# haiciyang/LaDiffCodec

Hardware: AMD Instinct MI355X
Metric: audio-sec decoded / wall-sec, 16kHz 3kbps 50-step DDPM (higher is better)
Workload: dtype bf16; 1 GPU; LaDiffCodec 3 kbps, diff_dims=256, enc_ratios 8 4, 50-step DDPM, batch=32x2.4 s utterances per GPU; global_batch=32, latent_len=1200, denoise_steps=50, rccl_ranks=1, batches_in_flight=1, parallelism=dp1 (utterance-sharded, no data-path collective)

## Files before the change

### ladiffcodec_amd/csrc/seanet.hip

```cpp
#include <type_traits>
#include "ldc_kernels.h"
#include "ldc_math.h"

namespace ldc {

__device__ __forceinline__ float sbf2f(unsigned short h) { return __uint_as_float(((unsigned)h) << 16); }
__device__ __forceinline__ unsigned short sf2bf(float f) { return hw_bf16(f); }
template <typename T>
__device__ __forceinline__ float sld(const void* p, size_t i);
template <>
__device__ __forceinline__ float sld<float>(const void* p, size_t i) { return reinterpret_cast<const float*>(p)[i]; }
template <>
__device__ __forceinline__ float sld<__bf16>(const void* p, size_t i) {
  return sbf2f(reinterpret_cast<const unsigned short*>(p)[i]);
}
template <typename T>
__device__ __forceinline__ void sst(void* p, size_t i, float v);
template <>
__device__ __forceinline__ void sst<float>(void* p, size_t i, float v) { reinterpret_cast<float*>(p)[i] = v; }
template <>
__device__ __forceinline__ void sst<__bf16>(void* p, size_t i, float v) {
  reinterpret_cast<unsigned short*>(p)[i] = sf2bf(v);
}

template <typename T>
__global__ __launch_bounds__(256) void conv_cin1_kernel(const float* x, void* y, const float* w, const float* bias,
                                                        int L, int Cout, int k) {
  extern __shared__ float sw[];
  for (int i = threadIdx.x; i < Cout * k; i += 256) sw[i] = w[i];
  for (int i = threadIdx.x; i < Cout; i += 256) sw[Cout * k + i] = bias ? bias[i] : 0.f;
  __syncthreads();
  const int b = blockIdx.y;
  const int pad = k - 1;
  const size_t total = (size_t)L * Cout;
  for (size_t idx = (size_t)blockIdx.x * 256 + threadIdx.x; idx < total; idx += (size_t)gridDim.x * 256) {
    const int l = (int)(idx / Cout), co = (int)(idx % Cout);
    float acc = sw[Cout * k + co];
    for (int t = 0; t < k; ++t) {
      int u = l + t - pad;
      if (u < 0) u = -u;
      if (u >= L) u = 2 * (L - 1) - u;
      acc += sw[co * k + t] * x[(size_t)b * L + u];
    }
    sst<T>(y, ((size_t)b * L + l) * Cout + co, acc);
  }
}

template <typename T>
__global__ __launch_bounds__(256) void conv_cin1_rows_kernel(const float* x, void* y, const float* w, const float* bias,
                                                             int L, int Cout, int k, int rows_per_block) {
  const int b = blockIdx.y;
  const int tpr = Cout / 4;
  const int c4 = (threadIdx.x % tpr) * 4, r0 = threadIdx.x / tpr, rstep = 256 / tpr;
  float wk[4][8], bv[4];
#pragma unroll
  for (int c = 0; c < 4; ++c) {
    bv[c] = bias ? bias[c4 + c] : 0.f;
#pragma unroll
    for (int t = 0; t < 8; ++t) wk[c][t] = t < k ? w[(c4 + c) * k + t] : 0.f;
  }
  const int pad = k - 1;
  const int lbeg = blockIdx.x * rows_per_block, lend = min(L, lbeg + rows_per_block);
  const float* xb = x + (size_t)b * L;
  for (int l = lbeg + r0; l < lend; l += rstep) {
    float xv[8];
#pragma unroll
    for (int t = 0; t < 8; ++t) {
      int u = l + t - pad;
      if (u < 0) u = -u;
      xv[t] = t < k ? xb[u] : 0.f;
    }
    float acc[4];
#pragma unroll
    for (int c = 0; c < 4; ++c) {
      acc[c] = bv[c];
#pragma unroll
      for (int t = 0; t < 8; ++t) acc[c] = fmaf(wk[c][t], xv[t], acc[c]);
    }
    const size_t o = ((size_t)b * L + l) * Cout + c4;
    if (sizeof(T) == 4) {
      *reinterpret_cast<float4*>(reinterpret_cast<float*>(y) + o) = make_float4(acc[0], acc[1], acc[2], acc[3]);
    } else {
      *reinterpret_cast<uint2*>(reinterpret_cast<unsigned short*>(y) + o) = make_uint2(hw_bf16x2(acc[0], acc[1]), hw_bf16x2(acc[2], acc[3]));
    }
  }
}

hipError_t launch_conv_cin1(int dt, const float* x, void* y, const float* w, const float* bias, int B, int L, int Cout,
                            int k, hipStream_t s, int* route_out) {
  if (L <= k - 1) return hipErrorInvalidValue;
  if (Cout % 4 == 0 && Cout <= 1024 && 256 % (Cout / 4) == 0 && k <= 8) {
    if (route_out) *route_out = CONV_ROUTE_CIN1_ROWS;
    const int rpb = 8 * (1024 / Cout);
    dim3 grid((L + rpb - 1) / rpb, B);
    if (dt == DT_F32) hipLaunchKernelGGL(conv_cin1_rows_kernel<float>, grid, dim3(256), 0, s, x, y, w, bias, L, Cout, k, rpb);
    else hipLaunchKernelGGL(conv_cin1_rows_kernel<__bf16>, grid, dim3(256), 0, s, x, y, w, bias, L, Cout, k, rpb);
    return hipGetLastError();
  }
  if (route_out) *route_out = CONV_ROUTE_CIN1_GENERIC;
  const size_t lds = (size_t)(Cout * k + Cout) * sizeof(float);
  int bx = (int)std::min<size_t>(((size_t)L * Cout + 255) / 256, 512);
  if (dt == DT_F32)
    hipLaunchKernelGGL(conv_cin1_kernel<float>, dim3(bx, B), dim3(256), lds, s, x, y, w, bias, L, Cout, k);
  else
    hipLaunchKernelGGL(conv_cin1_kernel<__bf16>, dim3(bx, B), dim3(256), lds, s, x, y, w, bias, L, Cout, k);
  return hipGetLastError();
}

__device__ __forceinline__ float sigmoid_acc(float v) { return 1.0f / (1.0f + expf(-v)); }

template <typename T, int H>
__global__ __launch_bounds__(4 * H) void lstm_reg_kernel(const void* pre, const float* w_hh, void* out, const void* skip,
                                                         const LstmSeq q) {
  constexpr int KS = H / 4;
  constexpr int KP = KS + 4;
  __shared__ __attribute__((aligned(16))) float sh[4 * KP];
  __shared__ float sg[4 * H];
  const int b = blockIdx.x, tid = threadIdx.x;
  const int rg = tid >> 2, g = tid & 3;
  float w[4][KS];
#pragma unroll
  for (int q = 0; q < 4; ++q)
#pragma unroll
    for (int k = 0; k < KS; k += 4) {
      const float4 v = *reinterpret_cast<const float4*>(w_hh + (size_t)(rg * 4 + q) * H + g * KS + k);
      w[q][k] = v.x; w[q][k + 1] = v.y; w[q][k + 2] = v.z; w[q][k + 3] = v.w;
    }
  const int row = tid;
  const bool resume = q.state && q.t0 > 0;
  float c = (resume && row < H) ? q.state[(size_t)b * 2 * H + H + row] : 0.f;
  float h_last = (resume && row < H) ? q.state[(size_t)b * 2 * H + row] : 0.f;
  if (row < H) sh[row + 4 * (row / KS)] = h_last;
  float p_next[4] = {0.f, 0.f, 0.f, 0.f};
  const size_t pre0 = (size_t)b * q.pre_bs, out0 = (size_t)b * q.out_bs, skip0 = (size_t)b * q.skip_bs;
  if (row < H) {
#pragma unroll
    for (int gq = 0; gq < 4; ++gq) p_next[gq] = sld<T>(pre, (pre0 + (size_t)q.t0 * q.pre_ts) * (4 * H) + gq * H + row);
  }
  float sk_next = (skip && row < H) ? sld<T>(skip, (skip0 + (size_t)q.t0 * q.skip_ts) * H + row) : 0.f;
  __syncthreads();
  for (int t = q.t0; t < q.t1; ++t) {
    const float p_cur[4] = {p_next[0], p_next[1], p_next[2], p_next[3]};
    const float sk = sk_next;
    if (t + 1 < q.t1 && row < H) {
#pragma unroll
      for (int gq = 0; gq < 4; ++gq) p_next[gq] = sld<T>(pre, (pre0 + (size_t)(t + 1) * q.pre_ts) * (4 * H) + gq * H + row);
      if (skip) sk_next = sld<T>(skip, (skip0 + (size_t)(t + 1) * q.skip_ts) * H + row);
    }
    typedef float f32x2 __attribute__((ext_vector_type(2)));
    f32x2 a01[4], a23[4];
#pragma unroll
    for (int q = 0; q < 4; ++q) { a01[q] = f32x2{0.f, 0.f}; a23[q] = f32x2{0.f, 0.f}; }
#pragma unroll
    for (int k = 0; k < KS; k += 4) {
      const float4 hv = *reinterpret_cast<const float4*>(&sh[g * KP + k]);
      const f32x2 h01 = {hv.x, hv.y}, h23 = {hv.z, hv.w};
#pragma unroll
      for (int q = 0; q < 4; ++q) {
        const f32x2 w01 = {w[q][k], w[q][k + 1]}, w23 = {w[q][k + 2], w[q][k + 3]};
        a01[q] = __builtin_elementwise_fma(w01, h01, a01[q]);
        a23[q] = __builtin_elementwise_fma(w23, h23, a23[q]);
      }
    }
#pragma unroll
    for (int q = 0; q < 4; ++q) {
      float v = (a01[q][0] + a01[q][1]) + (a23[q][0] + a23[q][1]);
      v += __int_as_float(__builtin_amdgcn_update_dpp(0, __float_as_int(v), 0xB1, 0xf, 0xf, true));
      v += __int_as_float(__builtin_amdgcn_update_dpp(0, __float_as_int(v), 0x4E, 0xf, 0xf, true));
      if (g == q) sg[rg * 4 + q] = v;
    }
    __syncthreads();
    if (row < H) {
      const float ig = fast_sigmoid(sg[row] + p_cur[0]), fg = fast_sigmoid(sg[H + row] + p_cur[1]);
      const float gg = fast_tanh(sg[2 * H + row] + p_cur[2]), og = fast_sigmoid(sg[3 * H + row] + p_cur[3]);
      c = fg * c + ig * gg;
      const float h = og * fast_tanh(c);
      h_last = h;
      sh[row + 4 * (row / KS)] = h;
      const size_t o = (out0 + (size_t)t * q.out_ts) * H + row;
      sst<T>(out, o, h + sk);
    }
    __syncthreads();
  }
  if (q.state && row < H) {
    q.state[(size_t)b * 2 * H + row] = h_last;
    q.state[(size_t)b * 2 * H + H + row] = c;
  }
}

template <typename T>
__global__ __launch_bounds__(1024) void lstm_stream_kernel(const void* pre, const float* w_km, void* out, const void* skip,
                                                           int T_len, int H) {
  extern __shared__ __attribute__((aligned(16))) float sm[];
  float* sh = sm;
  float* sg = sm + H;
  const int b = blockIdx.x, tid = threadIdx.x;
  const int G = 4 * H;
  for (int i = tid; i < H; i += 1024) sh[i] = 0.f;
  float c_state[4] = {0.f, 0.f, 0.f, 0.f};
  __syncthreads();
  for (int t = 0; t < T_len; ++t) {
    for (int row = tid; row < G; row += 1024) {
      float acc0 = 0.f, acc1 = 0.f;
      const float4* wp = reinterpret_cast<const float4*>(w_km) + row;
      for (int k4 = 0; k4 < H / 4; k4 += 2) {
        const float4 w0 = wp[(size_t)k4 * G];
        const float4 w1 = wp[(size_t)(k4 + 1) * G];
        const float4 h0 = *reinterpret_cast<const float4*>(&sh[4 * k4]);
        const float4 h1 = *reinterpret_cast<const float4*>(&sh[4 * k4 + 4]);
        acc0 += w0.x * h0.x + w0.y * h0.y + w0.z * h0.z + w0.w * h0.w;
        acc1 += w1.x * h1.x + w1.y * h1.y + w1.z * h1.z + w1.w * h1.w;
      }
      sg[row] = acc0 + acc1 + sld<T>(pre, ((size_t)b * T_len + t) * G + row);
    }
    __syncthreads();
    int ci = 0;
    for (int j = tid; j < H; j += 1024, ++ci) {
      const float ig = sigmoid_acc(sg[j]), fg = sigmoid_acc(sg[H + j]);
      const float gg = tanhf(sg[2 * H + j]), og = sigmoid_acc(sg[3 * H + j]);
      const float c = fg * c_state[ci] + ig * gg;
      c_state[ci] = c;
      const float h = og * tanhf(c);
      sh[j] = h;
      const size_t o = ((size_t)b * T_len + t) * H + j;
      sst<T>(out, o, skip ? h + sld<T>(skip, o) : h);
    }
    __syncthreads();
  }
}

constexpr int LSTM_COOP_SHARDS = 8;
constexpr int LSTM_COOP_SHARD_STRIDE = 16;
size_t lstm_coop_ws_bytes(int H) { return (size_t)2 * 32 * H * sizeof(float) + 256 * sizeof(unsigned); }

using f32x4 = __attribute__((ext_vector_type(4))) float;

template <typename T, int H>
__global__ __launch_bounds__(256) void lstm_coop_kernel(const void* pre, const float* w_hh, void* out, const void* skip,
                                                        int B, int T_len, float* hbuf, unsigned* sync, unsigned* host_flag) {
  constexpr int KW = H / 4;
  constexpr int NI = KW / 16;
  __shared__ float part[4][2][16][16];
  __shared__ int s_dead;
  const int tid = threadIdx.x, lane = tid & 63, w = tid >> 6;
  const int j = blockIdx.x, nb = gridDim.x;
  const int n = lane & 15, q = lane >> 4;
  const int MT = (B + 15) / 16;
  f32x4 breg[NI];
  {
    const size_t row = (size_t)(n >> 2) * H + 4 * j + (n & 3);
#pragma unroll
    for (int jj = 0; jj < NI; ++jj) breg[jj] = *reinterpret_cast<const f32x4*>(w_hh + row * H + w * KW + 16 * jj + 4 * q);
  }
  if (tid == 0) s_dead = 0;
  const int ob = tid >> 2, ou = tid & 3;
  const bool owner = tid < 4 * B;
  float c_state = 0.f;
  float pnext[4] = {0.f, 0.f, 0.f, 0.f};
  float sknext = 0.f;
  if (owner) {
#pragma unroll
    for (int g = 0; g < 4; ++g) pnext[g] = sld<T>(pre, ((size_t)ob * T_len) * (4 * H) + g * H + 4 * j + ou);
    if (skip) sknext = sld<T>(skip, ((size_t)ob * T_len) * H + 4 * j + ou);
  }
  __syncthreads();
  bool dead = false;
  int t = 0;
  for (; t < T_len; ++t) {
    f32x4 acc[2] = {{0.f, 0.f, 0.f, 0.f}, {0.f, 0.f, 0.f, 0.f}};
    if (t > 0) {
      if (w == 0) {
        const unsigned target = (unsigned)(t * (nb / LSTM_COOP_SHARDS));
        unsigned spins = 0;
        for (;;) {
          unsigned v = target;
          if (lane < LSTM_COOP_SHARDS) v = __hip_atomic_load(sync + lane * LSTM_COOP_SHARD_STRIDE, __ATOMIC_RELAXED, __HIP_MEMORY_SCOPE_AGENT);
          const unsigned flag = lane == 0 ? __hip_atomic_load(sync + 200, __ATOMIC_RELAXED, __HIP_MEMORY_SCOPE_AGENT) : 0u;
          if (__any(flag != 0u) || ++spins > 400000u) {
            if (lane == 0) { __hip_atomic_store(sync + 200, 1u, __ATOMIC_RELAXED, __HIP_MEMORY_SCOPE_AGENT); s_dead = 1; }
            break;
          }
          if (__all(v >= target)) break;
          __builtin_amdgcn_s_sleep(2);
        }
      }
      __syncthreads();
      if (s_dead) { dead = true; break; }
      const float* hp = hbuf + (size_t)((t + 1) & 1) * 32 * H;
      f32x4 areg[2][NI];
#pragma unroll
      for (int mt = 0; mt < 2; ++mt) {
        if (mt < MT) {
          const int item = min(mt * 16 + n, B - 1);
#pragma unroll
          for (int jj = 0; jj < NI; ++jj) {
            const float* src = hp + (size_t)item * H + w * KW + 16 * jj + 4 * q;
            asm volatile("global_load_dwordx4 %0, %1, off sc0 sc1" : "=v"(areg[mt][jj]) : "v"(src) : "memory");
          }
        }
      }
      asm volatile("s_waitcnt vmcnt(0)" ::: "memory");
#pragma unroll
      for (int mt = 0; mt < 2; ++mt)
        if (mt < MT) {
#pragma unroll
          for (int jj = 0; jj < NI; ++jj) asm volatile("" : "+v"(areg[mt][jj]));
        }
#pragma unroll
      for (int jj = 0; jj < NI; ++jj) {
#pragma unroll
        for (int e = 0; e < 4; ++e) {
          acc[0] = __builtin_amdgcn_mfma_f32_16x16x4f32(areg[0][jj][e], breg[jj][e], acc[0], 0, 0, 0);
          if (MT > 1) acc[1] = __builtin_amdgcn_mfma_f32_16x16x4f32(areg[1][jj][e], breg[jj][e], acc[1], 0, 0, 0);
        }
      }
    }
#pragma unroll
    for (int mt = 0; mt < 2; ++mt)
#pragma unroll
      for (int r = 0; r < 4; ++r) part[w][mt][4 * q + r][n] = acc[mt][r];
    __syncthreads();
    if (owner) {
      float gates[4];
#pragma unroll
      for (int g = 0; g < 4; ++g) {
        const int col = g * 4 + ou;
        gates[g] = pnext[g] + ((part[0][ob >> 4][ob & 15][col] + part[1][ob >> 4][ob & 15][col]) +
                               (part[2][ob >> 4][ob & 15][col] + part[3][ob >> 4][ob & 15][col]));
      }
      const float ig = sigmoid_acc(gates[0]), fg = sigmoid_acc(gates[1]);
      const float gg = tanhf(gates[2]), og = sigmoid_acc(gates[3]);
      c_state = fg * c_state + ig * gg;
      const float h = og * tanhf(c_state);
      __hip_atomic_store(hbuf + (size_t)(t & 1) * 32 * H + (size_t)ob * H + 4 * j + ou, h, __ATOMIC_RELAXED, __HIP_MEMORY_SCOPE_AGENT);
      asm volatile("s_waitcnt vmcnt(0)" ::: "memory");
      const size_t o = ((size_t)ob * T_len + t) * H + 4 * j + ou;
      sst<T>(out, o, h + sknext);
      if (t + 1 < T_len) {
#pragma unroll
        for (int g = 0; g < 4; ++g) pnext[g] = sld<T>(pre, ((size_t)ob * T_len + t + 1) * (4 * H) + g * H + 4 * j + ou);
        if (skip) sknext = sld<T>(skip, o + H);
      }
    }
    __syncthreads();
    if (tid == 0 && t + 1 < T_len)
      __hip_atomic_fetch_add(sync + (j % LSTM_COOP_SHARDS) * LSTM_COOP_SHARD_STRIDE, 1u, __ATOMIC_RELAXED, __HIP_MEMORY_SCOPE_AGENT);
  }
  if (dead && owner) {
    for (int tt = t; tt < T_len; ++tt) sst<T>(out, ((size_t)ob * T_len + tt) * H + 4 * j + ou, __builtin_nanf(""));
  }
  if (dead && tid == 0 && host_flag) __hip_atomic_store(host_flag, 1u, __ATOMIC_RELAXED, __HIP_MEMORY_SCOPE_SYSTEM);
}

template <int G>
__device__ __forceinline__ float dpp_sum_group(float v) {
  auto dpp = [](float x, auto ctrl) {
    return __int_as_float(__builtin_amdgcn_update_dpp(0, __float_as_int(x), decltype(ctrl)::value, 0xf, 0xf, true));
  };
  v += dpp(v, std::integral_constant<int, 0xB1>());
  v += dpp(v, std::integral_constant<int, 0x4E>());
  v += dpp(v, std::integral_constant<int, 0x141>());
  if (G >= 16) v += dpp(v, std::integral_constant<int, 0x140>());
  if (G >= 32) v += __shfl_xor(v, 16);
  if (G >= 64) v += __shfl_xor(v, 32);
  return v;
}

template <typename T, int H>
__global__ __launch_bounds__(1024) void lstm_xcd_kernel(const void* pre, const float* w_hh, void* out, const void* skip,
                                                        int B, int T_len, float* hbuf, unsigned* sync, unsigned* host_flag, unsigned long long* dbg = nullptr) {
  constexpr int NB = 16;
  constexpr int U = H / NB;
  constexpr int ROWS = 4 * U;
  constexpr int RPT = 2;
  constexpr int KSEG = 1024 / (ROWS / RPT);
  constexpr int KS = H / KSEG;
  constexpr int NV = KS / 4;
  constexpr int KPAD = KS >= 8 ? 4 : 0;
  __shared__ float sgate[2][ROWS];
  __shared__ __attribute__((aligned(16))) float sh[2][H + KPAD * KSEG];
  __shared__ int s_dead, s_rank;
  const int tid = threadIdx.x, lane = tid & 63, w = tid >> 6;
  const unsigned xcc = __builtin_amdgcn_s_getreg((20 << 0) | (0 << 6) | ((4 - 1) << 11)) & 7u;
  if (xcc != 0u) return;
  if (tid == 0) {
    s_rank = (int)__hip_atomic_fetch_add(sync + 202, 1u, __ATOMIC_RELAXED, __HIP_MEMORY_SCOPE_AGENT);
    s_dead = 0;
  }
  __syncthreads();
  const int j = s_rank;
  if (j >= NB) return;
  unsigned* flags = sync;
  const int rg = tid / KSEG, g = tid % KSEG;
  f32x4 wreg[RPT][NV];
#pragma unroll
  for (int q = 0; q < RPT; ++q) {
    const int r = rg * RPT + q;
    const size_t row = (size_t)(r / U) * H + (size_t)j * U + (r % U);
#pragma unroll
    for (int v = 0; v < NV; ++v) wreg[q][v] = *reinterpret_cast<const f32x4*>(w_hh + row * H + g * KS + 4 * v);
  }
  const int ob = tid / U, ou = tid % U;
  const bool owner = tid < U * B;
  float c_state = 0.f;
  float pnext[4] = {0.f, 0.f, 0.f, 0.f};
  float sknext = 0.f;
  if (owner) {
#pragma unroll
    for (int gg = 0; gg < 4; ++gg) pnext[gg] = sld<T>(pre, ((size_t)ob * T_len) * (4 * H) + gg * H + j * U + ou);
    if (skip) sknext = sld<T>(skip, ((size_t)ob * T_len) * H + j * U + ou);
  }
  bool dead = false;
  int t = 0;
  for (; t < T_len; ++t) {
    float dot[2][RPT];
#pragma unroll
    for (int q = 0; q < RPT; ++q) dot[0][q] = dot[1][q] = 0.f;
    unsigned long long st0 = 0, st1 = 0, st2 = 0, st3 = 0, st4 = 0, st5 = 0;
    const bool rec = dbg && j == 3 && tid == 0 && t >= 16 && t < 48;
    if (rec) st0 = __builtin_amdgcn_s_memtime();
    if (t > 0) {
      if (w == 0) {
        const unsigned long long t0 = wall_clock64();
        for (unsigned spins = 0;; ++spins) {
          const bool ok = lane >= NB || __hip_atomic_load(flags + lane, __ATOMIC_RELAXED, __HIP_MEMORY_SCOPE_AGENT) >= (unsigned)t;
          if (__all(ok)) break;
          if ((spins & 255u) == 255u) {
            const unsigned flag = lane == 0 ? __hip_atomic_load(sync + 200, __ATOMIC_RELAXED, __HIP_MEMORY_SCOPE_AGENT) : 0u;
            if (__any(flag != 0u) || wall_clock64() - t0 > 20000000ull) {
              if (lane == 0) { __hip_atomic_store(sync + 200, 1u, __ATOMIC_RELAXED, __HIP_MEMORY_SCOPE_AGENT); s_dead = 1; }
              break;
            }
          }
        }
      }
      __syncthreads();
      if (rec) st1 = __builtin_amdgcn_s_memtime();
      if (s_dead) { dead = true; break; }
      const float* hp = hbuf + (size_t)((t + 1) & 1) * 32 * H;
      if (tid < B * (H / 4)) {
        const int b = tid / (H / 4), v = tid % (H / 4);
        f32x4 hv;
        asm volatile("global_load_dwordx4 %0, %1, off sc1\n\ts_waitcnt vmcnt(0)" : "=&v"(hv) : "v"(hp + (size_t)b * H + 4 * v) : "memory");
        *reinterpret_cast<f32x4*>(&sh[b][4 * v + KPAD * ((4 * v) / KS)]) = hv;
      }
      __syncthreads();
      if (rec) st2 = __builtin_amdgcn_s_memtime();
#pragma unroll
      for (int b = 0; b < 2; ++b)
        if (b < B) {
#pragma unroll
          for (int v = 0; v < NV; ++v) {
            const f32x4 hv = *reinterpret_cast<const f32x4*>(&sh[b][g * (KS + KPAD) + 4 * v]);
#pragma unroll
            for (int q = 0; q < RPT; ++q)
#pragma unroll
              for (int e = 0; e < 4; ++e) dot[b][q] = fmaf(hv[e], wreg[q][v][e], dot[b][q]);
          }
        }
#pragma unroll
      for (int b = 0; b < 2; ++b)
        if (b < B) {
#pragma unroll
          for (int q = 0; q < RPT; ++q) dot[b][q] = dpp_sum_group<KSEG>(dot[b][q]);
        }
    }
    if (g == 0) {
#pragma unroll
      for (int q = 0; q < RPT; ++q) {
        sgate[0][rg * RPT + q] = dot[0][q];
        sgate[1][rg * RPT + q] = dot[1][q];
      }
    }
    __syncthreads();
    if (rec) st3 = __builtin_amdgcn_s_memtime();
    if (owner) {
      float gates[4];
#pragma unroll
      for (int gg = 0; gg < 4; ++gg) gates[gg] = pnext[gg] + sgate[ob][gg * U + ou];
      const float ig = sigmoid_acc(gates[0]), fg = sigmoid_acc(gates[1]);
      const float gv = tanhf(gates[2]), og = sigmoid_acc(gates[3]);
      c_state = fg * c_state + ig * gv;
      const float h = og * tanhf(c_state);
      asm volatile("global_store_dword %0, %1, off" ::"v"(hbuf + (size_t)(t & 1) * 32 * H + (size_t)ob * H + j * U + ou), "v"(h) : "memory");
      asm volatile("s_waitcnt vmcnt(0)" ::: "memory");
      if (rec) st4 = __builtin_amdgcn_s_memtime();
      const size_t o = ((size_t)ob * T_len + t) * H + j * U + ou;
      sst<T>(out, o, h + sknext);
      if (t + 1 < T_len) {
#pragma unroll
        for (int gg = 0; gg < 4; ++gg) pnext[gg] = sld<T>(pre, ((size_t)ob * T_len + t + 1) * (4 * H) + gg * H + j * U + ou);
        if (skip) sknext = sld<T>(skip, o + H);
      }
    }
    __syncthreads();
    if (tid == 0 && t + 1 < T_len) {
      asm volatile("global_store_dword %0, %1, off" ::"v"(flags + j), "v"((unsigned)(t + 1)) : "memory");
    }
    if (rec) { st5 = __builtin_amdgcn_s_memtime(); unsigned long long* o = dbg + (size_t)(t - 16) * 6; o[0] = st0; o[1] = st1; o[2] = st2; o[3] = st3; o[4] = st4; o[5] = st5; }
  }
  if (dead && owner) {
    for (int tt = t; tt < T_len; ++tt) sst<T>(out, ((size_t)ob * T_len + tt) * H + j * U + ou, __builtin_nanf(""));
  }
  if (dead && tid == 0 && host_flag) __hip_atomic_store(host_flag, 1u, __ATOMIC_RELAXED, __HIP_MEMORY_SCOPE_SYSTEM);
}

template <typename T>
static hipError_t lstm_coop_launch(const void* pre, const float* w_rm, void* out, const void* skip, int B, int T_len, int H,
                                   void* ws, unsigned* host_flag, int coop_launch, hipStream_t s) {
  float* hbuf = reinterpret_cast<float*>(ws);
  unsigned* sync = reinterpret_cast<unsigned*>(hbuf + (size_t)2 * 32 * H);
  const size_t esz = sizeof(T);
  for (int b0 = 0; b0 < B; b0 += 32) {
    const int nb = std::min(32, B - b0);
    hipError_t e = hipMemsetAsync(sync, 0, 256 * sizeof(unsigned), s);
    if (e != hipSuccess) return e;
    const char* p = reinterpret_cast<const char*>(pre) + (size_t)b0 * T_len * 4 * H * esz;
    char* o = reinterpret_cast<char*>(out) + (size_t)b0 * T_len * H * esz;
    const char* k = skip ? reinterpret_cast<const char*>(skip) + (size_t)b0 * T_len * H * esz : nullptr;
    const void* pp = p; void* oo = o; const void* kk = k; int nbv = nb, tl = T_len;
    void* args[] = {&pp, &w_rm, &oo, &kk, &nbv, &tl, &hbuf, &sync, &host_flag};
    const void* fn = H == 512 ? reinterpret_cast<const void*>(lstm_coop_kernel<T, 512>) : reinterpret_cast<const void*>(lstm_coop_kernel<T, 256>);
    if (coop_launch == 2 && nb <= 2) {
      const void* fx = H == 512 ? reinterpret_cast<const void*>(lstm_xcd_kernel<T, 512>) : reinterpret_cast<const void*>(lstm_xcd_kernel<T, 256>);
      static unsigned long long* dbg = nullptr;
      static int dbg_n = 0;
      if (getenv("LDC_LSTM_STAMPS") && !dbg) (void)hipMalloc((void**)&dbg, 32 * 6 * 8);
      void* args2[] = {&pp, &w_rm, &oo, &kk, &nbv, &tl, &hbuf, &sync, &host_flag, &dbg};
      e = hipLaunchKernel(fx, dim3(8 * 16), dim3(1024), args2, 0, s);
      if (dbg && ++dbg_n == 20) {
        (void)hipStreamSynchronize(s);
        unsigned long long hb[32 * 6];
        (void)hipMemcpy(hb, dbg, sizeof(hb), hipMemcpyDeviceToHost);
        double acc[6] = {0};
        for (int i = 1; i < 32; ++i) {
          acc[0] += (double)(hb[i * 6 + 1] - hb[i * 6 + 0]); acc[1] += (double)(hb[i * 6 + 2] - hb[i * 6 + 1]); acc[2] += (double)(hb[i * 6 + 3] - hb[i * 6 + 2]);
          acc[3] += (double)(hb[i * 6 + 4] - hb[i * 6 + 3]); acc[4] += (double)(hb[i * 6 + 5] - hb[i * 6 + 4]); acc[5] += (double)(hb[i * 6 + 0] - hb[(i - 1) * 6 + 0]);
        }
        fprintf(stderr, "[lstm_xcd] cycles per step: poll %.0f | h load %.0f | dot+reduce %.0f | gates+h store %.0f | rest+flag %.0f | step %.0f\n", acc[0] / 31, acc[1] / 31,
                acc[2] / 31, acc[3] / 31, acc[4] / 31, acc[5] / 31);
      }
    } else if (coop_launch == 1) e = hipLaunchCooperativeKernel(fn, dim3(H / 4), dim3(256), args, 0, s);
    else e = hipLaunchKernel(fn, dim3(H / 4), dim3(256), args, 0, s);
    if (e != hipSuccess) return e;
  }
  return hipSuccess;
}

bool lstm_coop_eligible(int H) { return H == 256 || H == 512; }
int lstm_xcd_resident(int H) {
  if (!lstm_coop_eligible(H)) return 0;
  const void* fn = H == 512 ? reinterpret_cast<const void*>(lstm_xcd_kernel<float, 512>) : reinterpret_cast<const void*>(lstm_xcd_kernel<float, 256>);
  int per_cu = 0, cus = 0, dev = 0;
  if (hipGetDevice(&dev) != hipSuccess || hipDeviceGetAttribute(&cus, hipDeviceAttributeMultiprocessorCount, dev) != hipSuccess ||
      hipOccupancyMaxActiveBlocksPerMultiprocessor(&per_cu, fn, 1024, 0) != hipSuccess) {
    (void)hipGetLastError();
    return 0;
  }
  if (cus % 8 != 0 || per_cu < 1) return 0;
  return per_cu * (cus / 8) / 16;
}

bool lstm_coop_resident(int H) {
  if (!lstm_coop_eligible(H)) return false;
  const void* fn = H == 512 ? reinterpret_cast<const void*>(lstm_coop_kernel<float, 512>) : reinterpret_cast<const void*>(lstm_coop_kernel<float, 256>);
  int dev = 0, per_cu = 0, cus = 0;
  if (hipGetDevice(&dev) != hipSuccess || hipDeviceGetAttribute(&cus, hipDeviceAttributeMultiprocessorCount, dev) != hipSuccess ||
      hipOccupancyMaxActiveBlocksPerMultiprocessor(&per_cu, fn, 256, 0) != hipSuccess) {
    (void)hipGetLastError();
    return false;
  }
  return (long long)std::max(0, per_cu - 1) * cus >= H / 4 || (long long)per_cu * cus >= 2 * (H / 4);
}

hipError_t launch_lstm_coop(int dt, const void* pre, const float* w_rm, void* out, const void* skip, int B, int T, int H,
                            void* ws, unsigned* host_flag, int coop_launch, hipStream_t s) {
  if (!lstm_coop_eligible(H)) return hipErrorInvalidValue;
  return dt == DT_F32 ? lstm_coop_launch<float>(pre, w_rm, out, skip, B, T, H, ws, host_flag, coop_launch, s)
                      : lstm_coop_launch<__bf16>(pre, w_rm, out, skip, B, T, H, ws, host_flag, coop_launch, s);
}

bool lstm_seq_supported(int H) { return H == 64 || H == 128; }

hipError_t launch_lstm_seq(int dt, const void* pre, const float* w_hh, void* out, const void* skip, int B, int H, const LstmSeq& q,
                           hipStream_t s) {
  if (!lstm_seq_supported(H) || q.t1 <= q.t0) return hipErrorInvalidValue;
  if (H == 64) {
    if (dt == DT_F32) hipLaunchKernelGGL((lstm_reg_kernel<float, 64>), dim3(B), dim3(256), 0, s, pre, w_hh, out, skip, q);
    else hipLaunchKernelGGL((lstm_reg_kernel<__bf16, 64>), dim3(B), dim3(256), 0, s, pre, w_hh, out, skip, q);
  } else {
    if (dt == DT_F32) hipLaunchKernelGGL((lstm_reg_kernel<float, 128>), dim3(B), dim3(512), 0, s, pre, w_hh, out, skip, q);
    else hipLaunchKernelGGL((lstm_reg_kernel<__bf16, 128>), dim3(B), dim3(512), 0, s, pre, w_hh, out, skip, q);
  }
  return hipGetLastError();
}

hipError_t launch_lstm_layer(int dt, const void* pre, const float* w_hh, void* out, const void* skip, int B, int T,
                             int H, hipStream_t s) {
  if (H % 8 || H > 4096) return hipErrorInvalidValue;
  if (H == 64 || H == 128) {
    LstmSeq q;
    q.t0 = 0; q.t1 = T; q.pre_bs = q.out_bs = q.skip_bs = T; q.pre_ts = q.out_ts = q.skip_ts = 1; q.state = nullptr;
    return launch_lstm_seq(dt, pre, w_hh, out, skip, B, H, q, s);
  } else {
    const size_t lds = (size_t)5 * H * sizeof(float);
    if (dt == DT_F32) hipLaunchKernelGGL(lstm_stream_kernel<float>, dim3(B), dim3(1024), lds, s, pre, w_hh, out, skip, T, H);
    else hipLaunchKernelGGL(lstm_stream_kernel<__bf16>, dim3(B), dim3(1024), lds, s, pre, w_hh, out, skip, T, H);
  }
  return hipGetLastError();
}

}
```

Measured before the change: 591.2 audio-s/wall-s.

## Remap LSTM gates per quad and double-buffer hidden state to drop a barrier

Reassigns the register-resident LSTM recurrent weights so each group of four lanes holds all four gates (i, f, g, o) of one hidden unit. The gate values are then exchanged with DPP quad broadcasts instead of going through a shared-memory gate buffer. The hidden state is double-buffered in LDS, which removes one of the two __syncthreads per timestep and the shared gate array. In exchange, all four lanes of a quad now compute the cell update redundantly, and the activation math is rewritten with a branch-free sigmoid/tanh that uses expf and a reciprocal.

```diff
diff --git a/ladiffcodec_amd/csrc/seanet.hip b/ladiffcodec_amd/csrc/seanet.hip
--- a/ladiffcodec_amd/csrc/seanet.hip
+++ b/ladiffcodec_amd/csrc/seanet.hip
@@ -114,38 +114,32 @@
                                                          const LstmSeq q) {
   constexpr int KS = H / 4;
   constexpr int KP = KS + 4;
-  __shared__ __attribute__((aligned(16))) float sh[4 * KP];
-  __shared__ float sg[4 * H];
+  __shared__ __attribute__((aligned(16))) float sh[2][4 * KP];
   const int b = blockIdx.x, tid = threadIdx.x;
-  const int rg = tid >> 2, g = tid & 3;
+  const int u = tid >> 2, g = tid & 3;
   float w[4][KS];
 #pragma unroll
   for (int q = 0; q < 4; ++q)
 #pragma unroll
     for (int k = 0; k < KS; k += 4) {
-      const float4 v = *reinterpret_cast<const float4*>(w_hh + (size_t)(rg * 4 + q) * H + g * KS + k);
+      const float4 v = *reinterpret_cast<const float4*>(w_hh + (size_t)(q * H + u) * H + g * KS + k);
       w[q][k] = v.x; w[q][k + 1] = v.y; w[q][k + 2] = v.z; w[q][k + 3] = v.w;
     }
-  const int row = tid;
   const bool resume = q.state && q.t0 > 0;
-  float c = (resume && row < H) ? q.state[(size_t)b * 2 * H + H + row] : 0.f;
-  float h_last = (resume && row < H) ? q.state[(size_t)b * 2 * H + row] : 0.f;
-  if (row < H) sh[row + 4 * (row / KS)] = h_last;
-  float p_next[4] = {0.f, 0.f, 0.f, 0.f};
+  float c = resume ? q.state[(size_t)b * 2 * H + H + u] : 0.f;
+  float h_last = resume ? q.state[(size_t)b * 2 * H + u] : 0.f;
+  if (g == 0) sh[0][u + 4 * (u / KS)] = h_last;
   const size_t pre0 = (size_t)b * q.pre_bs, out0 = (size_t)b * q.out_bs, skip0 = (size_t)b * q.skip_bs;
-  if (row < H) {
-#pragma unroll
-    for (int gq = 0; gq < 4; ++gq) p_next[gq] = sld<T>(pre, (pre0 + (size_t)q.t0 * q.pre_ts) * (4 * H) + gq * H + row);
-  }
-  float sk_next = (skip && row < H) ? sld<T>(skip, (skip0 + (size_t)q.t0 * q.skip_ts) * H + row) : 0.f;
+  float p_next = sld<T>(pre, (pre0 + (size_t)q.t0 * q.pre_ts) * (4 * H) + g * H + u);
+  float sk_next = (skip && g == 0) ? sld<T>(skip, (skip0 + (size_t)q.t0 * q.skip_ts) * H + u) : 0.f;
   __syncthreads();
-  for (int t = q.t0; t < q.t1; ++t) {
-    const float p_cur[4] = {p_next[0], p_next[1], p_next[2], p_next[3]};
+  int cur = 0;
+  for (int t = q.t0; t < q.t1; ++t, cur ^= 1) {
+    const float p_cur = p_next;
     const float sk = sk_next;
-    if (t + 1 < q.t1 && row < H) {
-#pragma unroll
-      for (int gq = 0; gq < 4; ++gq) p_next[gq] = sld<T>(pre, (pre0 + (size_t)(t + 1) * q.pre_ts) * (4 * H) + gq * H + row);
-      if (skip) sk_next = sld<T>(skip, (skip0 + (size_t)(t + 1) * q.skip_ts) * H + row);
+    if (t + 1 < q.t1) {
+      p_next = sld<T>(pre, (pre0 + (size_t)(t + 1) * q.pre_ts) * (4 * H) + g * H + u);
+      if (skip && g == 0) sk_next = sld<T>(skip, (skip0 + (size_t)(t + 1) * q.skip_ts) * H + u);
     }
     typedef float f32x2 __attribute__((ext_vector_type(2)));
     f32x2 a01[4], a23[4];
@@ -153,7 +147,7 @@
     for (int q = 0; q < 4; ++q) { a01[q] = f32x2{0.f, 0.f}; a23[q] = f32x2{0.f, 0.f}; }
 #pragma unroll
     for (int k = 0; k < KS; k += 4) {
-      const float4 hv = *reinterpret_cast<const float4*>(&sh[g * KP + k]);
+      const float4 hv = *reinterpret_cast<const float4*>(&sh[cur][g * KP + k]);
       const f32x2 h01 = {hv.x, hv.y}, h23 = {hv.z, hv.w};
 #pragma unroll
       for (int q = 0; q < 4; ++q) {
@@ -162,29 +156,33 @@
         a23[q] = __builtin_elementwise_fma(w23, h23, a23[q]);
       }
     }
+    float v[4];
 #pragma unroll
     for (int q = 0; q < 4; ++q) {
-      float v = (a01[q][0] + a01[q][1]) + (a23[q][0] + a23[q][1]);
-      v += __int_as_float(__builtin_amdgcn_update_dpp(0, __float_as_int(v), 0xB1, 0xf, 0xf, true));
-      v += __int_as_float(__builtin_amdgcn_update_dpp(0, __float_as_int(v), 0x4E, 0xf, 0xf, true));
-      if (g == q) sg[rg * 4 + q] = v;
+      v[q] = (a01[q][0] + a01[q][1]) + (a23[q][0] + a23[q][1]);
+      v[q] += __int_as_float(__builtin_amdgcn_update_dpp(0, __float_as_int(v[q]), 0xB1, 0xf, 0xf, true));
+      v[q] += __int_as_float(__builtin_amdgcn_update_dpp(0, __float_as_int(v[q]), 0x4E, 0xf, 0xf, true));
+    }
+    const float x = (g == 0 ? v[0] : g == 1 ? v[1] : g == 2 ? v[2] : v[3]) + p_cur;
+    const float e = __expf(g == 2 ? -2.0f * fabsf(x) : -x);
+    const float r = fast_rcp(1.0f + e);
+    const float act = g == 2 ? copysignf((1.0f - e) * r, x) : r;
+    const float ig = __int_as_float(__builtin_amdgcn_update_dpp(0, __float_as_int(act), 0x00, 0xf, 0xf, true));
+    const float fg = __int_as_float(__builtin_amdgcn_update_dpp(0, __float_as_int(act), 0x55, 0xf, 0xf, true));
+    const float gg = __int_as_float(__builtin_amdgcn_update_dpp(0, __float_as_int(act), 0xAA, 0xf, 0xf, true));
+    const float og = __int_as_float(__builtin_amdgcn_update_dpp(0, __float_as_int(act), 0xFF, 0xf, 0xf, true));
+    c = fg * c + ig * gg;
+    const float h = og * fast_tanh(c);
+    h_last = h;
+    if (g == 0) {
+      sh[cur ^ 1][u + 4 * (u / KS)] = h;
+      sst<T>(out, (out0 + (size_t)t * q.out_ts) * H + u, h + sk);
     }
     __syncthreads();
-    if (row < H) {
-      const float ig = fast_sigmoid(sg[row] + p_cur[0]), fg = fast_sigmoid(sg[H + row] + p_cur[1]);
-      const float gg = fast_tanh(sg[2 * H + row] + p_cur[2]), og = fast_sigmoid(sg[3 * H + row] + p_cur[3]);
-      c = fg * c + ig * gg;
-      const float h = og * fast_tanh(c);
-      h_last = h;
-      sh[row + 4 * (row / KS)] = h;
-      const size_t o = (out0 + (size_t)t * q.out_ts) * H + row;
-      sst<T>(out, o, h + sk);
-    }
-    __syncthreads();
-  }
-  if (q.state && row < H) {
-    q.state[(size_t)b * 2 * H + row] = h_last;
-    q.state[(size_t)b * 2 * H + H + row] = c;
+  }
+  if (q.state && g == 0) {
+    q.state[(size_t)b * 2 * H + u] = h_last;
+    q.state[(size_t)b * 2 * H + H + u] = c;
   }
 }
 
```

New measurement: 591.7 audio-s/wall-s (median of 3 runs). Within noise of the previous version (+0.1%).
